# Chthi/Ofighters

Measured on AMD Instinct MI355X. Metric: arena-steps/sec (env.step+obs+policy fwd) at 4096 arenas, 1/2/4/8 MI355X, higher is better.
Workload: dtype f32; 1 GPU; 4096 arenas x 8 ships per GPU, random-bot actions + step + 2D obs rasterise (u8 maps) + bi-head policy forward for 8 ship(s)/arena, trunk shared per arena (BASELINE configs[3]); arenas_per_gpu=4096, ships=8, laser_cap=512, episode_ticks=200, parallelism=arena-sharded x1, RCCL all-reduce of episodic scores only, laser_overflow=0, last_episode_score_sum=70993, last_episode_arenas=4096

## Files before the change

ofighters_amd/csrc/ofx_head.hip:

```cpp
#include "ofx_head.h"
#include "ofx_lowp.h"
#include "ofx_diag.h"
#include <stdlib.h>


typedef float f32x4 __attribute__((ext_vector_type(4)));
typedef float f32x2 __attribute__((ext_vector_type(2)));
#define HD_PS 400
constexpr int HC4_ZERO = 800;
constexpr int HC4_COL = 816, HC4_CPITCH = 416;
constexpr int HC4_STRIDE = HC4_COL + 2 * HC4_CPITCH + 16;
__device__ __forceinline__ int hc4_at(int ln, int t) { return ln < 2 ? ln * 400 + t : HC4_COL + (ln - 2) * HC4_CPITCH + t; }
__device__ __forceinline__ int hc4_pad(int k) { return k < 16 ? HC4_ZERO + k : k < 32 ? HC4_COL + 400 + k - 16 : HC4_COL + HC4_CPITCH + 400 + k - 32; }

__device__ __forceinline__ void hc4_zero_block(const HeadParams2 &p, int tid, int threads) {
  if (blockIdx.x == 0)
    for (int e = tid; e < HC4_STRIDE; e += threads) p.c4[(size_t)p.S * HC4_STRIDE + e] = 0.f;
}

__device__ __forceinline__ float hd_max_raw(float x, float floor) {
  float pinf;
  asm("s_mov_b32 %0, 0x7f800000" : "=s"(pinf));
  return __builtin_amdgcn_fmed3f(x, floor, pinf);
}
// ... 182 lines not shown
    float acc = 0.f;
    if (!isc || (t > 0 && t < 399)) {
      const int d0 = side ? 2 : 0;
#pragma unroll
      for (int d1 = 0; d1 < 3; d1++)
#pragma unroll
        for (int ci = 0; ci < 8; ci++) {
          const int tap = isc ? d1 * 3 + d0 : d0 * 3 + d1;
          acc += p.w4raw[tap * 8 + ci] * hf_up(u3l + ln * 1600 + ci, 8, 200, t + d1 - 1, p.legacy);
        }
      if (!isc && (t == 0 || t == 399)) {
        const int cl = t ? 3 : 2, dx = t ? 2 : 0;
        for (int dy = 0; dy < 3; dy++) {
          if (dy == d0) continue;
          const int yy = (side ? 399 : 0) + dy - 1;
          if (yy < 0 || yy > 399) continue;
          for (int ci = 0; ci < 8; ci++) acc += p.w4raw[(dy * 3 + dx) * 8 + ci] * hf_up(u3l + cl * 1600 + ci, 8, 200, yy, p.legacy);
        }
      }
    }
    p.c4[(size_t)s * HC4_STRIDE + hc4_at(ln, t)] = acc;
  }
  if (tid < 64) p.c4[(size_t)s * HC4_STRIDE + hc4_pad(tid)] = 0.f;
}

constexpr int HG_THREADS = 256;
constexpr int HG_L1 = 0;
constexpr int HG_U3 = 0;
constexpr int HG_RB = 6400;
constexpr int HG_CB = HG_RB + 4 * 102 * 4;
constexpr int HG_TOTAL = HG_CB + 4 * 102 * 4;
static_assert(2 * 52 * 52 <= 6400, "l1p fits under u3l");

template <int CIN, int COUT, class G>
__device__ __forceinline__ float hg_corner(G get, int n, int yc, int xc, const float *w, float bias, int co, int legacy) {
  float acc = bias;
  for (int dy = 0; dy < 3; dy++) {
    const int uy = yc + dy - 1;
    if (uy < 0 || uy >= 2 * n) continue;
    int ya, yb; float wy;
    hf_taps(uy, n, ya, yb, wy, legacy);
    for (int dx = 0; dx < 3; dx++) {
      const int ux = xc + dx - 1;
      if (ux < 0 || ux >= 2 * n) continue;
      int xa, xb; float wx;
      hf_taps(ux, n, xa, xb, wx, legacy);
      for (int ci = 0; ci < CIN; ci++) {
        const float a = get(ya, xa, ci), b = get(ya, xb, ci), d = get(yb, xa, ci), g = get(yb, xb, ci);
        const float top = a + (b - a) * wx, bot = d + (g - d) * wx;
        acc += w[((dy * 3 + dx) * CIN + ci) * COUT + co] * (top + (bot - top) * wy);
      }
    }
  }
  return fmaxf(acc, 0.f);
}

__global__ __launch_bounds__(HG_THREADS) void k_head_frames(HeadParams2 p) {
  __shared__ __align__(16) float sm[HG_TOTAL];
  __shared__ float efr_s[192], w4s[72];
  const int s = hd_ship(p, (int)((blockIdx.x & ~7u) | ((blockIdx.x + (blockIdx.x >> 3)) & 7u)));
  const int tid = threadIdx.x, lane = tid & 63;
  hc4_zero_block(p, tid, HG_THREADS);
  if (s < 0) return;
  const int wv = __builtin_amdgcn_readfirstlane(tid >> 6);
  const int n16 = lane & 15, kq = lane >> 4;
  float *l1p = sm + HG_L1, *u2rb = sm + HG_RB, *u2cb = sm + HG_CB, *u3l = sm + HG_U3;

  {
    constexpr int NB = 6 * 52 + 46 * 6, NE = 2 * NB, PER = (NE + HG_THREADS - 1) / HG_THREADS;
    float v[PER];
    int at[PER];
#pragma unroll
    for (int u = 0; u < PER; u++) {
      const int e = min(u * HG_THREADS + tid, NE - 1);
      const int ci = e / NB, k = e - ci * NB;
      int r, c;
      if (k < 6 * 52) { const int rr = k / 52; r = rr < 3 ? rr : rr + 46; c = k - rr * 52; }
      else { const int k2 = k - 6 * 52, cc = k2 % 6; r = 3 + k2 / 6; c = cc < 3 ? cc : cc + 46; }
      at[u] = (ci * 52 + r) * 52 + c;
      v[u] = p.up1[(size_t)s * 5000 + (ci * 50 + min(max(r - 1, 0), 49)) * 50 + min(max(c - 1, 0), 49)];
    }
#pragma unroll
    for (int u = 0; u < PER; u++)
      if (u * HG_THREADS + tid < NE) l1p[at[u]] = v[u];
  }
  if (tid < 192) efr_s[tid] = p.efr[tid];
  if (tid < 72) w4s[tid] = p.w4raw[tid];
  __syncthreads();

  float bw2[5];
#pragma unroll
  for (int jj = 0; jj < 5; jj++) bw2[jj] = p.w2fr[(wv * 20 + 4 * jj + kq) * 16 + n16];
  float bw3[9];
#pragma unroll
  for (int jj = 0; jj < 9; jj++) bw3[jj] = p.w3fr[(wv * 36 + 4 * jj + kq) * 16 + n16];
#pragma unroll 1
  for (int m = 0; m < 4; m++) {
    const int v = wv;
    const int pp = min(16 * m + n16, 49);
    const int i = v == 0 ? 0 : v == 1 ? 49 : pp, j = v == 2 ? 0 : v == 3 ? 49 : pp;
    const float bias = p.b2[n16 & 3];
    f32x4 d = {bias, bias, bias, bias};
#pragma unroll
    for (int jj = 0; jj < 5; jj++) {
      const int tap = min(2 * jj + (kq >> 1), 8);
      const float a = l1p[((kq & 1) * 52 + i + tap / 3) * 52 + j + tap % 3];
      d = __builtin_amdgcn_mfma_f32_16x16x4f32(a, bw2[jj], d, 0, 0, 0);
    }
    const int co = n16 & 3, pa = n16 >> 3, pb = (n16 >> 2) & 1;
#pragma unroll
    for (int r = 0; r < 4; r++) {
      const int q = 16 * m + 4 * kq + r;
      if (q >= 50) continue;
      const float val = fmaxf(d[r], 0.f);
      if (v < 2) {
        u2rb[((2 * v + pa) * 102 + 2 * q + pb + 1) * 4 + co] = val;
      } else {
        u2cb[((2 * (v - 2) + pb) * 102 + 2 * q + pa + 1) * 4 + co] = val;
      }
    }
  }
  __syncthreads();
  if (tid < 64) {
    const int co = tid & 3, cx = (tid >> 2) & 1, cy = (tid >> 3) & 1, bx = (tid >> 4) & 1, by = tid >> 5;
    const int y = by ? 98 + cy : cy, x = bx ? 98 + cx : cx;
    const int rb = by ? 2 + cy : cy, cb = bx ? 2 + cx : cx;
    const bool fy = y == 0 || y == 99, fx = x == 0 || x == 99;
    float val;
    if (fy && fx) {
      auto get = [&](int yy, int xx, int ci) { return l1p[(ci * 52 + yy + 1) * 52 + xx + 1]; };
      val = hg_corner<2, 4>(get, 50, y, x, p.w2raw, p.b2[co], co, p.legacy);
    } else if (fx) {
      val = u2cb[(cb * 102 + y + 1) * 4 + co];
    } else {
      val = u2rb[(rb * 102 + x + 1) * 4 + co];
    }
    if (fy && fx) { u2rb[(rb * 102 + x + 1) * 4 + co] = val; u2cb[(cb * 102 + y + 1) * 4 + co] = val; }
    else if (fx) u2rb[(rb * 102 + x + 1) * 4 + co] = val;
    else u2cb[(cb * 102 + y + 1) * 4 + co] = val;
  }
  __syncthreads();
  if (tid < 128) {
    const int co = tid & 3, b = (tid >> 2) & 3, hi = (tid >> 4) & 1, isc = tid >> 5;
    if (isc < 2) {
      float *ln = (isc ? u2cb : u2rb) + b * 102 * 4;
      ln[(hi ? 101 : 0) * 4 + co] = ln[(hi ? 100 : 1) * 4 + co];
    }
  }
  for (int e = tid; e < 4 * 100 * 4; e += HG_THREADS) {
    const int ln = e / 400, r = e - ln * 400;
    const float *src = ln < 2 ? u2rb + (ln ? 3 : 0) * 408 : u2cb + (ln == 3 ? 3 : 0) * 408;
    p.u2fr[(size_t)s * 1600 + e] = src[4 + r];
  }
  __syncthreads();

#pragma unroll 1
  for (int m = 0; m < 7; m++) {
    const int v = wv;
    const int qq = min(16 * m + n16, 99);
    const float *band = (v < 2 ? u2rb : u2cb);
    const int b0 = (v & 1) ? 2 : 0;
    const float bias = p.b3[n16 & 7];
    f32x4 d = {bias, bias, bias, bias};
#pragma unroll
    for (int jj = 0; jj < 9; jj++) {
      const int ty = jj / 3, tx = jj % 3;
      const int tf = v < 2 ? ty : tx, ta = v < 2 ? tx : ty;
      const int bsel = (v & 1) ? b0 + min(tf, 1) : b0 + max(tf - 1, 0);
      const float a = band[(bsel * 102 + qq + ta) * 4 + kq];
      d = __builtin_amdgcn_mfma_f32_16x16x4f32(a, bw3[jj], d, 0, 0, 0);
    }
    const int co = n16 & 7, par = n16 >> 3;
#pragma unroll
    for (int r = 0; r < 4; r++) {
      const int q = 16 * m + 4 * kq + r;
      if (q < 100) u3l[(v * 200 + 2 * q + par) * 8 + co] = fmaxf(d[r], 0.f);
    }
  }
  __syncthreads();
  if (tid < 32) {
    const int co = tid & 7, c = tid >> 3;
    const int y = (c & 1) ? 199 : 0, x = (c & 2) ? 199 : 0;
    auto get = [&](int yy, int xx, int ci) {
      return u2rb[((yy < 50 ? yy : yy - 96) * 102 + xx + 1) * 4 + ci];
    };
    const float val = hg_corner<4, 8>(get, 100, y, x, p.w3raw, p.b3[co], co, p.legacy);
    u3l[(((c & 1) ? 1 : 0) * 200 + x) * 8 + co] = val;
    u3l[(((c & 2) ? 3 : 2) * 200 + y) * 8 + co] = val;
  }
  __syncthreads();
  if (tid < 252) {
    const int tp = tid % 9, c0 = tid / 9;
    float wt[8];
#pragma unroll
    for (int ci = 0; ci < 8; ci++) wt[ci] = w4s[tp * 8 + ci];
    float *dst = p.vfr + (size_t)s * 7200 + tid;
    for (int cell = c0; cell < 4 * 200; cell += 28) {
      const f32x4 ua = *reinterpret_cast<const f32x4 *>(u3l + cell * 8), ub = *reinterpret_cast<const f32x4 *>(u3l + cell * 8 + 4);
      float acc = 0.f;
#pragma unroll
      for (int ci = 0; ci < 4; ci++) acc = fmaf(wt[ci], ua[ci], acc);
#pragma unroll
      for (int ci = 0; ci < 4; ci++) acc = fmaf(wt[4 + ci], ub[ci], acc);
      dst[(cell - c0) * 9] = acc;
    }
  }

  for (int e = tid; e < 4 * 400; e += HG_THREADS) {
    const int ln = e / 400, t = e - ln * 400, isc = ln >> 1, side = ln & 1, jq = t >> 1, b = t & 1;
    float acc = 0.f;
    if (!isc || (t > 0 && t < 399)) {
      const float *E = efr_s + ((isc * 2 + side) * 2 + b) * 24;
      const float *L = u3l + ln * 1600;
#pragma unroll
      for (int o = 0; o < 3; o++) {
        const float *Lp = L + min(max(jq + o - 1, 0), 199) * 8;
#pragma unroll
        for (int ci = 0; ci < 8; ci++) acc += E[o * 8 + ci] * Lp[ci];
      }
      if (!isc && (t == 0 || t == 399)) {
        const int cs = t ? 1 : 0;
        const int yq = side ? 199 : 0, a = side ? 1 : 0;
        const float *E2 = efr_s + ((2 + cs) * 2 + a) * 24;
        const float *L2 = u3l + (2 + cs) * 1600;
        for (int o = 0; o < 3; o++) {
          const float *Lp = L2 + min(max(yq + o - 1, 0), 199) * 8;
          for (int ci = 0; ci < 8; ci++) acc += E2[o * 8 + ci] * Lp[ci];
        }
        const int tap = (side ? 2 : 0) * 3 + (cs ? 2 : 0);
        const float *Lc = L + (t ? 199 : 0) * 8;
        for (int ci = 0; ci < 8; ci++) acc -= p.w4raw[tap * 8 + ci] * Lc[ci];
      }
    }
    p.c4[(size_t)s * HC4_STRIDE + hc4_at(ln, t)] = acc;
  }
  if (tid < 64) p.c4[(size_t)s * HC4_STRIDE + hc4_pad(tid)] = 0.f;
}

constexpr int HS_GPR = 13;
constexpr int HS_NTILES = 325;
constexpr int HS_NS = 42;
constexpr int HS_NR3 = 16, HS_P3 = 106;
constexpr int HS_PL3 = HS_NR3 * HS_P3 + 4;
constexpr int HS_NV = 9;
constexpr int HS_NR2 = 16, HS_P2 = 56;
constexpr int HS_PL2 = (HS_NR2 + 2) * HS_P2;
static_assert(HS_PL2 % 32 == 16, "uprelu2 plane stride");
constexpr int HS_TABP = 16 * HS_GPR;
static_assert(HS_TABP == 4 * 52, "table period in tiles");
static_assert(4 * (HS_NV * HS_PL3 + 4 * HS_PL2 + HS_TABP + 400) <= 80 * 1024, "two workgroups per CU");
struct alignas(16) HsPick { signed char v[HS_NS][4]; };
constexpr int hs_pairs_done_c(int s) { return s + 2 + ((s + 2) >> 2) < 50 ? s + 2 + ((s + 2) >> 2) : 50; }
constexpr HsPick hs_make_pick() {
  HsPick t{};
  for (int st = 0; st < HS_NS; st++)
    for (int cw = 0; cw < 4; cw++) {
      const int lo = 2 * hs_pairs_done_c(st), hi = 2 * hs_pairs_done_c(st + 1);
      const int at = lo + ((cw - lo) & 3);
      t.v[st][cw] = (signed char)(at < hi ? at >> 1 : -1);
    }
  return t;
}
__constant__ HsPick kHsPick = hs_make_pick();

// ... 558 lines not shown
```

ofighters_amd/csrc/ofx_policy.hip:

```cpp
#include <string.h>

#include "ofx_internal.h"
#include "ofx_blob.h"
#include "ofx_trunk.h"
#include "ofx_head.h"

typedef float f32x16 __attribute__((ext_vector_type(16)));


extern "C" int ofx_policy_layout(const ofx_handle *h, ofx_policy_desc *desc) {
  (void)h;
  if (!desc) { ofx_set_error("ofx_policy_layout: null desc"); return OFX_ERR_INVALID; }
  memset(desc, 0, sizeof(*desc));
  desc->n_tensors = policy_layout(desc->offset, desc->count);
  desc->n_floats = desc->offset[desc->n_tensors];
  return OFX_OK;
}

struct PrepLayout {
  int tw[4], tb[4];
  int uw[3], ub[3];
  int w3mf;
  int w2mf;
  int w2fr;
  int w3fr;
  int w4eff_c;
  int w4raw;
  int efr;
  int b4;
  int zero16;
  int wbm[3];
  int lut1;
  int total;
};

static PrepLayout prep_layout() {
  PrepLayout L;
  int off = 0;
  for (int i = 0; i < 4; i++) { L.tw[i] = off; off += 9 * kTrunkCin[i] * 8; L.tb[i] = off; off += 8; }
  for (int i = 0; i < 3; i++) { L.uw[i] = off; off += 9 * kUpCin[i] * kUpCout[i]; L.ub[i] = off; off += kUpCout[i]; }
// ... 147 lines not shown
      p.prep[p.dst_wbm[l - 1] + e] = (tr >= 0 && tr < 3) ? p.prep[p.dst_w[l] + ((tr * 3 + dx) * 8 + ci) * 8 + co] : 0.f;
    }
  }
}

__global__ __launch_bounds__(256) void k_upconv1(ConvParams p) {
  __shared__ float u0s[625];
  __shared__ float up[52][53];
  const int tid = threadIdx.x;
  const int n_items = p.live ? p.live[0] : p.images;
#pragma unroll 1
  for (int it = blockIdx.x; it < n_items; it += gridDim.x) {
  const int img = p.live ? p.live[1 + it] : it;
  __syncthreads();
  for (int e = tid; e < 625; e += 256) u0s[e] = p.in[(size_t)img * 625 + e];
  __syncthreads();
  for (int e = tid; e < 52 * 52; e += 256) {
    const int c = e % 52, r = e / 52, gy = r - 1, gx = c - 1;
    float v = 0.f;
    if (gy >= 0 && gy < 50 && gx >= 0 && gx < 50) {
      const float sy = p.legacy ? (float)gy * 0.5f : ((float)gy + 0.5f) * 0.5f - 0.5f;
      const float sx = p.legacy ? (float)gx * 0.5f : ((float)gx + 0.5f) * 0.5f - 0.5f;
      const float fy = floorf(sy), fx = floorf(sx);
      const float ly = sy - fy, lx = sx - fx;
      int y0 = (int)fy, x0 = (int)fx, y1 = y0 + 1, x1 = x0 + 1;
      y0 = max(y0, 0); x0 = max(x0, 0); y1 = min(y1, 24); x1 = min(x1, 24);
      const float a = u0s[y0 * 25 + x0], b = u0s[y0 * 25 + x1], d = u0s[y1 * 25 + x0], g = u0s[y1 * 25 + x1];
      const float top = a + (b - a) * lx, bot = d + (g - d) * lx;
      v = top + (bot - top) * ly;
    }
    up[r][c] = v;
  }
  __syncthreads();
  if (tid < 250) {
  const int row = tid / 5, x0 = 10 * (tid - 5 * row);
  float acc[2][10];
#pragma unroll
  for (int co = 0; co < 2; co++)
#pragma unroll
    for (int i = 0; i < 10; i++) acc[co][i] = 0.f;
#pragma unroll
  for (int dy = 0; dy < 3; dy++) {
    float v[12];
#pragma unroll
    for (int i = 0; i < 12; i++) v[i] = up[row + dy][x0 + i];
#pragma unroll
    for (int dx = 0; dx < 3; dx++)
#pragma unroll
      for (int co = 0; co < 2; co++) {
        const float wv = p.w[(dy * 3 + dx) * 2 + co];
#pragma unroll
        for (int i = 0; i < 10; i++) acc[co][i] = __builtin_fmaf(v[i + dx], wv, acc[co][i]);
      }
  }
#pragma unroll
  for (int co = 0; co < 2; co++) {
    const float bias = p.b[co];
    float *o = p.out + (((size_t)img * 2 + co) * 50 + row) * 50 + x0;
#pragma unroll
    for (int i = 0; i < 10; i += 2)
      *reinterpret_cast<float2 *>(o + i) = make_float2(fmaxf(acc[co][i] + bias, 0.f), fmaxf(acc[co][i + 1] + bias, 0.f));
  }
  }
  }
}


__global__ __launch_bounds__(256) void k_gemm_f32(const float *A, int lda, const float *B, int ldb, const float *bias,
                                                  float *C, int ldc, int M, int N, int K, int relu, const int32_t *live) {
  const int lane = threadIdx.x & 63, wv = threadIdx.x >> 6;
  const int tiles_n = (N + 31) / 32;
  const int tile = blockIdx.x * 4 + wv;
  if (live) M = live[0];
  if (tile >= ((M + 31) / 32) * tiles_n) return;
  const int m0 = (tile / tiles_n) * 32, n0 = (tile % tiles_n) * 32;
  const int r0 = m0 + (lane & 31), c = n0 + (lane & 31), kh = lane >> 5;
  const bool rv = r0 < M, cv = c < N;
  const int r = live ? live[1 + (rv ? r0 : 0)] : r0;
  f32x16 acc;
#pragma unroll
  for (int i = 0; i < 16; i++) acc[i] = 0.f;
  const float *ap = A + (size_t)(rv ? r : 0) * lda + kh;
  const float *bp = B + (size_t)kh * ldb + (cv ? c : 0);
  for (int k0 = 0; k0 < K; k0 += 2) {
    const bool kv = k0 + kh < K;
    const float a = (rv && kv) ? ap[k0] : 0.f;
    const float b = (cv && kv) ? bp[(size_t)k0 * ldb] : 0.f;
    acc = __builtin_amdgcn_mfma_f32_32x32x2f32(a, b, acc, 0, 0, 0);
  }
  if (cv) {
    const float bv = bias ? bias[c] : 0.f;
#pragma unroll
    for (int i = 0; i < 16; i++) {
      const int row = m0 + (i & 3) + 8 * (i >> 2) + 4 * kh;
      if (row < M) {
        float v = acc[i] + bv;
        if (relu) v = fmaxf(v, 0.f);
        C[(size_t)(live ? live[1 + row] : row) * ldc + c] = v;
      }
    }
  }
}

__global__ __launch_bounds__(256) void k_gemm_f32_splitk(const float *A, int lda, const float *B, int ldb, float *P,
                                                         int M, int N, int Kc, int tiles, int jobs) {
  const int lane = threadIdx.x & 63, wv = threadIdx.x >> 6;
  const int tiles_n = (N + 31) / 32;
  const int job = blockIdx.x * 4 + wv;
  const int chunk = job / tiles, tile = job - chunk * tiles;
  if (job >= jobs) return;
  const int m0 = (tile / tiles_n) * 32, n0 = (tile % tiles_n) * 32;
  const int r = m0 + (lane & 31), c = n0 + (lane & 31), kh = lane >> 5;
  const bool rv = r < M, cv = c < N;
  f32x16 acc;
#pragma unroll
  for (int i = 0; i < 16; i++) acc[i] = 0.f;
  const float *ap = A + (size_t)(rv ? r : 0) * lda + (size_t)chunk * Kc + 4 * kh;
  const float *bp = B + ((size_t)chunk * Kc + 4 * kh) * ldb + (cv ? c : 0);
  for (int k0 = 0; k0 < Kc; k0 += 8) {
    const float4 a4 = *reinterpret_cast<const float4 *>(ap + k0);
    const float b0 = bp[(size_t)(k0 + 0) * ldb], b1 = bp[(size_t)(k0 + 1) * ldb], b2 = bp[(size_t)(k0 + 2) * ldb],
                b3 = bp[(size_t)(k0 + 3) * ldb];
    acc = __builtin_amdgcn_mfma_f32_32x32x2f32(rv ? a4.x : 0.f, cv ? b0 : 0.f, acc, 0, 0, 0);
    acc = __builtin_amdgcn_mfma_f32_32x32x2f32(rv ? a4.y : 0.f, cv ? b1 : 0.f, acc, 0, 0, 0);
    acc = __builtin_amdgcn_mfma_f32_32x32x2f32(rv ? a4.z : 0.f, cv ? b2 : 0.f, acc, 0, 0, 0);
    acc = __builtin_amdgcn_mfma_f32_32x32x2f32(rv ? a4.w : 0.f, cv ? b3 : 0.f, acc, 0, 0, 0);
  }
  if (cv) {
    float *out = P + (size_t)chunk * M * N;
#pragma unroll
    for (int i = 0; i < 16; i++) {
      const int row = m0 + (i & 3) + 8 * (i >> 2) + 4 * kh;
      if (row < M) out[(size_t)row * N + c] = acc[i];
    }
  }
}

struct HeadParams {
  int N, M;
  ofx_state st;
  const float *g1;
  int g1_chunks;
  const float *k1, *b1, *k2, *b2, *k3, *b3;
  const int32_t *live;
  const uint8_t *mask;
  const float *vec8;
  float *d1;
  float *act;
  int32_t *iaction;
};

__global__ __launch_bounds__(256) void k_head_dense(HeadParams p) {
  __shared__ float sd1[4][100];
  __shared__ float sd2[4][50];
  const int lane = threadIdx.x & 63, wv = threadIdx.x >> 6;
  const int item = blockIdx.x * 4 + wv, n_items = p.live ? p.live[0] : p.N * p.M;
  if ((int)blockIdx.x * 4 >= n_items) return;
  const bool on = item < n_items;
  const int s = on ? (p.live ? p.live[1 + item] : item) : 0;
  const int a = s / p.M;
  float vec[8];
  if (on) {
    if (p.vec8) {
#pragma unroll
      for (int k = 0; k < 8; k++) vec[k] = p.vec8[(size_t)s * 8 + k];
    } else {
      vec[0] = (float)p.st.reward[s]; vec[1] = 1.f;
      vec[2] = (float)p.st.ship_px[s]; vec[3] = (float)p.st.ship_py[s];
      vec[4] = (float)PS; vec[5] = (float)PS;
      vec[6] = (float)p.st.ship_x[s]; vec[7] = (float)p.st.ship_y[s];
    }
    for (int o = lane; o < 100; o += 64) {
      float acc = 0.f;
#pragma unroll
      for (int k = 0; k < 8; k++) acc += vec[k] * p.k1[k * 100 + o];
      float g = 0.f;
      for (int ch = 0; ch < p.g1_chunks; ch++) g += p.g1[((size_t)ch * p.N + a) * 100 + o];
      acc += g;
      acc += p.b1[o];
      acc = fmaxf(acc, 0.f);
      sd1[wv][o] = acc;
      p.d1[(size_t)s * 100 + o] = acc;
    }
  }
  __syncthreads();
  if (on && lane < 50) {
    float acc = 0.f;
    for (int k = 0; k < 100; k++) acc += sd1[wv][k] * p.k2[k * 50 + lane];
    sd2[wv][lane] = fmaxf(acc + p.b2[lane], 0.f);
  }
  __syncthreads();
  if (on && lane < 2) {
    float acc = 0.f;
    for (int k = 0; k < 50; k++) acc += sd2[wv][k] * p.k3[k * 2 + lane];
    acc += p.b3[lane];
    if (p.act) p.act[(size_t)s * 2 + lane] = acc;
    const float other = __shfl_xor(acc, 1);
    if (lane == 0 && p.iaction) p.iaction[s] = other > acc ? 1 : 0;
  }
}

__device__ inline float unordered_f32(unsigned o) {
  return __uint_as_float((o & 0x80000000u) ? (o & 0x7FFFFFFFu) : ~o);
}

__global__ void k_policy_finish(int S, const uint8_t *mask, const unsigned long long *best, int32_t *ipointer,
                                float *ptr_max) {
  const int s = blockIdx.x * blockDim.x + threadIdx.x;
  if (s >= S || (mask && !mask[s])) return;
  const bool none = best[s] == 0ull;
  const unsigned k = none ? 0u : ~(unsigned)(best[s] & 0xFFFFFFFFull);
  ipointer[2 * s] = (int)(k % PS);
  ipointer[2 * s + 1] = (int)(k / PS);
  if (ptr_max) ptr_max[s] = none ? __builtin_nanf("") : unordered_f32((unsigned)(best[s] >> 32));
}

__global__ void k_policy_actions(int S, const ofx_state st, const int32_t *iaction, const int32_t *ipointer,
                                 const uint8_t *mask, ofx_action *out) {
  const int s = blockIdx.x * blockDim.x + threadIdx.x;
  if (s >= S || (mask && !mask[s])) return;
  ofx_action a;
  a.valid = st.alive[s] ? 1 : 0;
  a.shoot = iaction[s] == 0;
  a.thrust = iaction[s] == 1;
  a.px = ipointer[2 * s];
  a.py = ipointer[2 * s + 1];
  a._pad = 0;
  out[s] = a;
}

struct PolicyWs {
// ... 120 lines not shown
  float *act_values, *heatmap, *ptr_max, *ptr_probe;
  int32_t *iaction, *ipointer;
  const int32_t *probe;
};

static int policy_forward_impl(ofx_handle *h, const ForwardArgs &a) {
  const int N = a.N, S = a.N * a.M;
  const float *weights = a.weights;
  PolicyWs ws;
  int rc = policy_workspace(h, &ws, N, S);
  if (rc) return rc;
  int32_t off[64], cnt[64];
  policy_layout(off, cnt);
  const PrepLayout L = prep_layout();

  const bool pinned = h->prep && h->prep_pinned == weights;
  if (!pinned && (rc = policy_prepare(h, weights, &h->prep_tmp))) return rc;
  const float *prep = pinned ? h->prep : h->prep_tmp;

  const int lowp = a.vec8 == nullptr ? h->opt_policy_lowp : 0;
  TrunkParams tp;
  memset(&tp, 0, sizeof(tp));
  tp.bits[0] = a.bits[0]; tp.bits[1] = a.bits[1]; tp.bits_stride = a.bits_stride; tp.images = N;
  for (int i = 0; i < 4; i++) { tp.tw[i] = prep + L.tw[i]; tp.tb[i] = prep + L.tb[i]; }
  for (int i = 0; i < 3; i++) tp.wbm[i] = prep + L.wbm[i];
  tp.lut1 = prep + L.lut1; tp.zero16 = prep + L.zero16;
  tp.p1 = ws.p1; tp.p2 = ws.p2; tp.p3 = ws.p3; tp.p4 = ws.p4;
  tp.lowp = lowp; tp.sparse = h->opt_trunk_sparse || a.vec8 != nullptr;
  tp.stat = h->opt_trunk_sparse ? h->trunk_stat : nullptr;
  if ((rc = ofx_launch_trunk(h, tp))) return rc;

  const float *k1 = weights + off[OFX_T_DENSE1];
  {
    const int tiles = ((N + 31) / 32) * 4, jobs = tiles * kDense1Chunks;
    hipLaunchKernelGGL(k_gemm_f32_splitk, dim3((jobs + 3) / 4), dim3(256), 0, h->stream, ws.p4, 5000, k1 + 8 * 100, 100,
                       ws.g1, N, 100, 5000 / kDense1Chunks, tiles, jobs);
    OFX_HIP(hipGetLastError());
  }
  HeadParams hp;
  hp.N = N; hp.M = a.M; hp.st = h->st; hp.vec8 = a.vec8; hp.g1 = ws.g1; hp.g1_chunks = kDense1Chunks;
  hp.k1 = k1; hp.b1 = weights + off[OFX_T_DENSE1 + 1];
  hp.k2 = weights + off[OFX_T_DENSE2]; hp.b2 = weights + off[OFX_T_DENSE2 + 1];
  hp.k3 = weights + off[OFX_T_OUT1]; hp.b3 = weights + off[OFX_T_OUT1 + 1];
  const int32_t *live = nullptr;
  if (a.ship_mask) {
    if ((rc = ofx_head_compact(h, S, a.ship_mask, ws.live))) return rc;
    live = ws.live;
  }
  hp.mask = a.ship_mask; hp.live = live; hp.d1 = ws.d1; hp.act = a.act_values; hp.iaction = a.iaction ? a.iaction : ws.iaction;
  hipLaunchKernelGGL(k_head_dense, dim3((S + 3) / 4), dim3(256), 0, h->stream, hp);
  OFX_HIP(hipGetLastError());

  if ((rc = ofx_launch_gemm(h, ws.d1, 100, weights + off[OFX_T_UPDENSE], 625, weights + off[OFX_T_UPDENSE + 1], ws.u0, 625, S, 625, 100, 1, live)))
    return rc;
  ConvParams up;
  memset(&up, 0, sizeof(up));
  up.live = live; up.images = S; up.legacy = h->opt_bilinear_legacy;
  up.in = ws.u0; up.w = prep + L.uw[0]; up.b = prep + L.ub[0]; up.out = ws.up1;
  hipLaunchKernelGGL(k_upconv1, dim3((unsigned)(live && S > 4096 ? 4096 : S)), dim3(256), 0, h->stream, up);
  OFX_HIP(hipGetLastError());
  OFX_HIP(hipMemsetAsync(ws.best, 0, sizeof(unsigned long long) * S, h->stream));
  HeadParams2 hp2;
  memset(&hp2, 0, sizeof(hp2));
  hp2.S = S; hp2.up1 = ws.up1;
  hp2.w2mf = prep + L.w2mf; hp2.b2 = prep + L.ub[1]; hp2.w2raw = prep + L.uw[1];
  hp2.w3mf = prep + L.w3mf; hp2.b3 = prep + L.ub[2]; hp2.w3raw = prep + L.uw[2];
  hp2.w4eff_c = prep + L.w4eff_c; hp2.b4 = prep + L.b4; hp2.w4raw = prep + L.w4raw;
  hp2.w2fr = prep + L.w2fr; hp2.w3fr = prep + L.w3fr; hp2.efr = prep + L.efr;
  hp2.u2fr = ws.u2fr; hp2.vfr = ws.vfr; hp2.c4 = ws.c4;
  hp2.frames_ref = h->opt_frames_ref; hp2.legacy = h->opt_bilinear_legacy;
  hp2.bf16 = lowp;
  hp2.mask = a.ship_mask; hp2.live = ws.live; hp2.live_ready = a.ship_mask != nullptr; hp2.best = ws.best; hp2.heat = a.heatmap;
  hp2.probe = a.probe; hp2.ptr_probe = a.probe ? a.ptr_probe : nullptr;
  const int pb = h->prof_base;
  hp2.event_base = pb;
  if ((rc = ofx_launch_head(h, hp2))) return rc;
  if (pb >= 0) h->prof_base = pb + 3 < OFX_RING_MAX ? pb + 2 : -1;
  hipLaunchKernelGGL(k_policy_finish, dim3((S + 255) / 256), dim3(256), 0, h->stream, S, a.ship_mask, ws.best,
                     a.ipointer ? a.ipointer : ws.ipointer, a.ptr_max);
  OFX_HIP(hipGetLastError());
  return OFX_OK;
}

extern "C" int ofx_policy_forward(ofx_handle *h, const float *weights, const uint8_t *ship_mask, float *act_values,
                                  int32_t *iaction, int32_t *ipointer, float *heatmap) {
  if (!h || !weights) { ofx_set_error("ofx_policy_forward: null argument"); return OFX_ERR_INVALID; }
  if (!h->spawned) { ofx_set_error("You must execute analyse_battleground first."); return OFX_ERR_STATE; }
  const ofx_config &c = h->cfg;
  if (c.width != PS || c.height != PS) {
    ofx_set_error("ofx_policy_forward: the pointer_model takes 400x400 maps (got %d x %d)", c.width, c.height);
    return OFX_ERR_INVALID;
  }
  OFX_HIP(hipSetDevice(c.device));
  int rc = ofx_launch_raster(h, OFX_MAP_BITS_LSB, nullptr, nullptr);
// ... 92 lines not shown
```

Measured before the change: 221,200 arena-steps/s.

## Restructure policy head GEMMs, dense head batching and head-frames MFMA loops

Rewrites the dense1 split-K GEMM to stage 64-row A tiles in LDS with register-prefetched B, and moves the chunk reduction into its own small kernel. Replaces the generic up-dense GEMM launch with a dedicated K=100 MFMA kernel that keeps A rows in LDS. Each k_head_dense wave now handles 8 ships, which reuses weight loads across them. Zeroing of `best` moves into that kernel, replacing a separate memset. Head-frames code interleaves two MFMA tiles per iteration, preloads corner weights into registers, reads w4 from LDS, and remaps upconv1 threads to cover all 256 lanes. The cost is more launches, higher register and LDS pressure, and `best` is now zeroed only for live ships.

```diff
diff --git a/ofighters_amd/csrc/ofx_head.hip b/ofighters_amd/csrc/ofx_head.hip
--- a/ofighters_amd/csrc/ofx_head.hip
+++ b/ofighters_amd/csrc/ofx_head.hip
@@ -238,23 +238,35 @@
 constexpr int HG_TOTAL = HG_CB + 4 * 102 * 4;
 static_assert(2 * 52 * 52 <= 6400, "l1p fits under u3l");
 
+template <int CIN, int COUT>
+__device__ __forceinline__ void hg_corner_w(float (&wt)[4 * CIN], int yc, int xc, const float *w, int co) {
+  const int dy0 = yc == 0 ? 1 : 0, dx0 = xc == 0 ? 1 : 0;
+#pragma unroll
+  for (int t = 0; t < 2; t++)
+#pragma unroll
+    for (int u = 0; u < 2; u++)
+#pragma unroll
+      for (int ci = 0; ci < CIN; ci++) wt[(t * 2 + u) * CIN + ci] = w[(((dy0 + t) * 3 + dx0 + u) * CIN + ci) * COUT + co];
+}
 template <int CIN, int COUT, class G>
-__device__ __forceinline__ float hg_corner(G get, int n, int yc, int xc, const float *w, float bias, int co, int legacy) {
+__device__ __forceinline__ float hg_corner(G get, int n, int yc, int xc, const float (&wt)[4 * CIN], float bias, int legacy) {
+  const int dy0 = yc == 0 ? 1 : 0, dx0 = xc == 0 ? 1 : 0;
   float acc = bias;
-  for (int dy = 0; dy < 3; dy++) {
-    const int uy = yc + dy - 1;
-    if (uy < 0 || uy >= 2 * n) continue;
+#pragma unroll
+  for (int t = 0; t < 2; t++) {
+    const int uy = yc + dy0 + t - 1;
     int ya, yb; float wy;
     hf_taps(uy, n, ya, yb, wy, legacy);
-    for (int dx = 0; dx < 3; dx++) {
-      const int ux = xc + dx - 1;
-      if (ux < 0 || ux >= 2 * n) continue;
+#pragma unroll
+    for (int u = 0; u < 2; u++) {
+      const int ux = xc + dx0 + u - 1;
       int xa, xb; float wx;
       hf_taps(ux, n, xa, xb, wx, legacy);
+#pragma unroll
       for (int ci = 0; ci < CIN; ci++) {
         const float a = get(ya, xa, ci), b = get(ya, xb, ci), d = get(yb, xa, ci), g = get(yb, xb, ci);
         const float top = a + (b - a) * wx, bot = d + (g - d) * wx;
-        acc += w[((dy * 3 + dx) * CIN + ci) * COUT + co] * (top + (bot - top) * wy);
+        acc += wt[(t * 2 + u) * CIN + ci] * (top + (bot - top) * wy);
       }
     }
   }
@@ -292,39 +304,63 @@
   }
   if (tid < 192) efr_s[tid] = p.efr[tid];
   if (tid < 72) w4s[tid] = p.w4raw[tid];
-  __syncthreads();
-
   float bw2[5];
 #pragma unroll
   for (int jj = 0; jj < 5; jj++) bw2[jj] = p.w2fr[(wv * 20 + 4 * jj + kq) * 16 + n16];
   float bw3[9];
 #pragma unroll
   for (int jj = 0; jj < 9; jj++) bw3[jj] = p.w3fr[(wv * 36 + 4 * jj + kq) * 16 + n16];
+  const float bias2 = p.b2[n16 & 3], bias3 = p.b3[n16 & 7];
+  float wc2[8], wc3[16], bc2 = 0.f, bc3 = 0.f;
+#pragma unroll
+  for (int e = 0; e < 8; e++) wc2[e] = 0.f;
+#pragma unroll
+  for (int e = 0; e < 16; e++) wc3[e] = 0.f;
+  if (tid < 64 && ((tid >> 3) & 1) == (tid >> 5) && ((tid >> 2) & 1) == ((tid >> 4) & 1)) {
+    hg_corner_w<2, 4>(wc2, (tid >> 5) ? 99 : 0, ((tid >> 4) & 1) ? 99 : 0, p.w2raw, tid & 3);
+    bc2 = p.b2[tid & 3];
+  }
+  if (tid < 32) {
+    hg_corner_w<4, 8>(wc3, ((tid >> 3) & 1) ? 199 : 0, ((tid >> 3) & 2) ? 199 : 0, p.w3raw, tid & 7);
+    bc3 = p.b3[tid & 7];
+  }
+  __syncthreads();
+
 #pragma unroll 1
-  for (int m = 0; m < 4; m++) {
+  for (int m0 = 0; m0 < 4; m0 += 2) {
     const int v = wv;
-    const int pp = min(16 * m + n16, 49);
-    const int i = v == 0 ? 0 : v == 1 ? 49 : pp, j = v == 2 ? 0 : v == 3 ? 49 : pp;
-    const float bias = p.b2[n16 & 3];
-    f32x4 d = {bias, bias, bias, bias};
+    f32x4 d[2];
+    int ai[2];
+#pragma unroll
+    for (int c = 0; c < 2; c++) {
+      const int pp = min(16 * (m0 + c) + n16, 49);
+      const int i = v == 0 ? 0 : v == 1 ? 49 : pp, j = v == 2 ? 0 : v == 3 ? 49 : pp;
+      ai[c] = ((kq & 1) * 52 + i) * 52 + j;
+      d[c] = f32x4{bias2, bias2, bias2, bias2};
+    }
 #pragma unroll
     for (int jj = 0; jj < 5; jj++) {
       const int tap = min(2 * jj + (kq >> 1), 8);
-      const float a = l1p[((kq & 1) * 52 + i + tap / 3) * 52 + j + tap % 3];
-      d = __builtin_amdgcn_mfma_f32_16x16x4f32(a, bw2[jj], d, 0, 0, 0);
+#pragma unroll
+      for (int c = 0; c < 2; c++) {
+        const float a = l1p[ai[c] + (tap / 3) * 52 + tap % 3];
+        d[c] = __builtin_amdgcn_mfma_f32_16x16x4f32(a, bw2[jj], d[c], 0, 0, 0);
+      }
     }
     const int co = n16 & 3, pa = n16 >> 3, pb = (n16 >> 2) & 1;
 #pragma unroll
-    for (int r = 0; r < 4; r++) {
-      const int q = 16 * m + 4 * kq + r;
-      if (q >= 50) continue;
-      const float val = fmaxf(d[r], 0.f);
-      if (v < 2) {
-        u2rb[((2 * v + pa) * 102 + 2 * q + pb + 1) * 4 + co] = val;
-      } else {
-        u2cb[((2 * (v - 2) + pb) * 102 + 2 * q + pa + 1) * 4 + co] = val;
-      }
-    }
+    for (int c = 0; c < 2; c++)
+#pragma unroll
+      for (int r = 0; r < 4; r++) {
+        const int q = 16 * (m0 + c) + 4 * kq + r;
+        if (q >= 50) continue;
+        const float val = fmaxf(d[c][r], 0.f);
+        if (v < 2) {
+          u2rb[((2 * v + pa) * 102 + 2 * q + pb + 1) * 4 + co] = val;
+        } else {
+          u2cb[((2 * (v - 2) + pb) * 102 + 2 * q + pa + 1) * 4 + co] = val;
+        }
+      }
   }
   __syncthreads();
   if (tid < 64) {
@@ -335,7 +371,7 @@
     float val;
     if (fy && fx) {
       auto get = [&](int yy, int xx, int ci) { return l1p[(ci * 52 + yy + 1) * 52 + xx + 1]; };
-      val = hg_corner<2, 4>(get, 50, y, x, p.w2raw, p.b2[co], co, p.legacy);
+      val = hg_corner<2, 4>(get, 50, y, x, wc2, bc2, p.legacy);
     } else if (fx) {
       val = u2cb[(cb * 102 + y + 1) * 4 + co];
     } else {
@@ -361,27 +397,31 @@
   __syncthreads();
 
 #pragma unroll 1
-  for (int m = 0; m < 7; m++) {
+  for (int m0 = 0; m0 < 8; m0 += 2) {
     const int v = wv;
-    const int qq = min(16 * m + n16, 99);
     const float *band = (v < 2 ? u2rb : u2cb);
     const int b0 = (v & 1) ? 2 : 0;
-    const float bias = p.b3[n16 & 7];
-    f32x4 d = {bias, bias, bias, bias};
+    f32x4 d[2] = {f32x4{bias3, bias3, bias3, bias3}, f32x4{bias3, bias3, bias3, bias3}};
 #pragma unroll
     for (int jj = 0; jj < 9; jj++) {
       const int ty = jj / 3, tx = jj % 3;
       const int tf = v < 2 ? ty : tx, ta = v < 2 ? tx : ty;
       const int bsel = (v & 1) ? b0 + min(tf, 1) : b0 + max(tf - 1, 0);
-      const float a = band[(bsel * 102 + qq + ta) * 4 + kq];
-      d = __builtin_amdgcn_mfma_f32_16x16x4f32(a, bw3[jj], d, 0, 0, 0);
+#pragma unroll
+      for (int c = 0; c < 2; c++) {
+        const int qq = min(16 * (m0 + c) + n16, 99);
+        const float a = band[(bsel * 102 + qq + ta) * 4 + kq];
+        d[c] = __builtin_amdgcn_mfma_f32_16x16x4f32(a, bw3[jj], d[c], 0, 0, 0);
+      }
     }
     const int co = n16 & 7, par = n16 >> 3;
 #pragma unroll
-    for (int r = 0; r < 4; r++) {
-      const int q = 16 * m + 4 * kq + r;
-      if (q < 100) u3l[(v * 200 + 2 * q + par) * 8 + co] = fmaxf(d[r], 0.f);
-    }
+    for (int c = 0; c < 2; c++)
+#pragma unroll
+      for (int r = 0; r < 4; r++) {
+        const int q = 16 * (m0 + c) + 4 * kq + r;
+        if (q < 100) u3l[(v * 200 + 2 * q + par) * 8 + co] = fmaxf(d[c][r], 0.f);
+      }
   }
   __syncthreads();
   if (tid < 32) {
@@ -390,7 +430,7 @@
     auto get = [&](int yy, int xx, int ci) {
       return u2rb[((yy < 50 ? yy : yy - 96) * 102 + xx + 1) * 4 + ci];
     };
-    const float val = hg_corner<4, 8>(get, 100, y, x, p.w3raw, p.b3[co], co, p.legacy);
+    const float val = hg_corner<4, 8>(get, 100, y, x, wc3, bc3, p.legacy);
     u3l[(((c & 1) ? 1 : 0) * 200 + x) * 8 + co] = val;
     u3l[(((c & 2) ? 3 : 2) * 200 + y) * 8 + co] = val;
   }
@@ -435,7 +475,7 @@
         }
         const int tap = (side ? 2 : 0) * 3 + (cs ? 2 : 0);
         const float *Lc = L + (t ? 199 : 0) * 8;
-        for (int ci = 0; ci < 8; ci++) acc -= p.w4raw[tap * 8 + ci] * Lc[ci];
+        for (int ci = 0; ci < 8; ci++) acc -= w4s[tap * 8 + ci] * Lc[ci];
       }
     }
     p.c4[(size_t)s * HC4_STRIDE + hc4_at(ln, t)] = acc;
diff --git a/ofighters_amd/csrc/ofx_policy.hip b/ofighters_amd/csrc/ofx_policy.hip
--- a/ofighters_amd/csrc/ofx_policy.hip
+++ b/ofighters_amd/csrc/ofx_policy.hip
@@ -6,6 +6,8 @@
 #include "ofx_head.h"
 
 typedef float f32x16 __attribute__((ext_vector_type(16)));
+typedef float f32x4 __attribute__((ext_vector_type(4)));
+typedef float f32x2 __attribute__((ext_vector_type(2)));
 
 
 extern "C" int ofx_policy_layout(const ofx_handle *h, ofx_policy_desc *desc) {
@@ -219,35 +221,30 @@
     up[r][c] = v;
   }
   __syncthreads();
-  if (tid < 250) {
-  const int row = tid / 5, x0 = 10 * (tid - 5 * row);
-  float acc[2][10];
-#pragma unroll
-  for (int co = 0; co < 2; co++)
-#pragma unroll
-    for (int i = 0; i < 10; i++) acc[co][i] = 0.f;
-#pragma unroll
-  for (int dy = 0; dy < 3; dy++) {
-    float v[12];
-#pragma unroll
-    for (int i = 0; i < 12; i++) v[i] = up[row + dy][x0 + i];
-#pragma unroll
-    for (int dx = 0; dx < 3; dx++)
-#pragma unroll
-      for (int co = 0; co < 2; co++) {
-        const float wv = p.w[(dy * 3 + dx) * 2 + co];
-#pragma unroll
-        for (int i = 0; i < 10; i++) acc[co][i] = __builtin_fmaf(v[i + dx], wv, acc[co][i]);
-      }
-  }
-#pragma unroll
-  for (int co = 0; co < 2; co++) {
-    const float bias = p.b[co];
-    float *o = p.out + (((size_t)img * 2 + co) * 50 + row) * 50 + x0;
-#pragma unroll
-    for (int i = 0; i < 10; i += 2)
-      *reinterpret_cast<float2 *>(o + i) = make_float2(fmaxf(acc[co][i] + bias, 0.f), fmaxf(acc[co][i + 1] + bias, 0.f));
-  }
+#pragma unroll 1
+  for (int e = tid; e < 1250; e += 256) {
+    const int row = e / 25, x0 = 2 * (e - 25 * row);
+    float acc[2][2] = {{0.f, 0.f}, {0.f, 0.f}};
+#pragma unroll
+    for (int dy = 0; dy < 3; dy++) {
+      float v[4];
+#pragma unroll
+      for (int i = 0; i < 4; i++) v[i] = up[row + dy][x0 + i];
+#pragma unroll
+      for (int dx = 0; dx < 3; dx++)
+#pragma unroll
+        for (int co = 0; co < 2; co++) {
+          const float wv = p.w[(dy * 3 + dx) * 2 + co];
+#pragma unroll
+          for (int i = 0; i < 2; i++) acc[co][i] = __builtin_fmaf(v[i + dx], wv, acc[co][i]);
+        }
+    }
+#pragma unroll
+    for (int co = 0; co < 2; co++) {
+      const float bias = p.b[co];
+      *reinterpret_cast<float2 *>(p.out + ((size_t)img * 2 + co) * 2500 + 2 * e) =
+          make_float2(fmaxf(acc[co][0] + bias, 0.f), fmaxf(acc[co][1] + bias, 0.f));
+    }
   }
   }
 }
@@ -289,45 +286,172 @@
   }
 }
 
+constexpr int AR_P = 52;
+template <int K, int NT>
+__device__ __forceinline__ void gemm_arows_tiles(const float *ar, const float *B, int ldb, const float *bias, float *C,
+                                                 int ldc, int M, int N, int relu, const int32_t *live, int m0, int lane, int t0) {
+  const int kh = lane >> 5;
+  f32x16 acc[NT];
+  const float *bp[NT];
+  bool cv[NT];
+#pragma unroll
+  for (int q = 0; q < NT; q++) {
+    const int c = (t0 + 4 * q) * 32 + (lane & 31);
+    cv[q] = c < N;
+    bp[q] = B + (size_t)kh * ldb + (cv[q] ? c : 0);
+#pragma unroll
+    for (int i = 0; i < 16; i++) acc[q][i] = 0.f;
+  }
+#pragma unroll 2
+  for (int i4 = 0; i4 < K / 8; i4++) {
+    const f32x4 x = *reinterpret_cast<const f32x4 *>(ar + 4 * i4);
+#pragma unroll
+    for (int u = 0; u < 4; u++)
+#pragma unroll
+      for (int q = 0; q < NT; q++) {
+        const float b = cv[q] ? bp[q][(size_t)(2 * u) * ldb] : 0.f;
+        acc[q] = __builtin_amdgcn_mfma_f32_32x32x2f32(x[u], b, acc[q], 0, 0, 0);
+      }
+#pragma unroll
+    for (int q = 0; q < NT; q++) bp[q] += (size_t)8 * ldb;
+  }
+  {
+    const f32x2 x = *reinterpret_cast<const f32x2 *>(ar + 4 * (K / 8));
+#pragma unroll
+    for (int u = 0; u < 2; u++)
+#pragma unroll
+      for (int q = 0; q < NT; q++) {
+        const float b = cv[q] ? bp[q][(size_t)(2 * u) * ldb] : 0.f;
+        acc[q] = __builtin_amdgcn_mfma_f32_32x32x2f32(x[u], b, acc[q], 0, 0, 0);
+      }
+  }
+#pragma unroll
+  for (int q = 0; q < NT; q++) {
+    if (!cv[q]) continue;
+    const int c = (t0 + 4 * q) * 32 + (lane & 31);
+    const float bv = bias ? bias[c] : 0.f;
+#pragma unroll
+    for (int i = 0; i < 16; i++) {
+      const int row = m0 + (i & 3) + 8 * (i >> 2) + 4 * kh;
+      if (row < M) {
+        float v = acc[q][i] + bv;
+        if (relu) v = fmaxf(v, 0.f);
+        C[(size_t)(live ? live[1 + row] : row) * ldc + c] = v;
+      }
+    }
+  }
+}
+
+template <int K>
+__global__ __launch_bounds__(256) __attribute__((amdgpu_waves_per_eu(4, 4)))
+void k_gemm_f32_arows(const float *A, int lda, const float *B, int ldb, const float *bias, float *C, int ldc, int M, int N,
+                      int relu, const int32_t *live) {
+  static_assert(K % 8 == 4 && K / 2 + 2 <= AR_P, "k_gemm_f32_arows: K");
+  __shared__ __align__(16) float sA[2 * 32 * AR_P];
+  const int tid = threadIdx.x, lane = tid & 63, wv = __builtin_amdgcn_readfirstlane(tid >> 6);
+  if (live) M = live[0];
+  const int m0 = blockIdx.x * 32;
+  if (m0 >= M) return;
+  {
+    constexpr int Q = K / 4, NE = 32 * Q, PER = (NE + 255) / 256;
+    float4 v[PER];
+#pragma unroll
+    for (int u = 0; u < PER; u++) {
+      const int e = min(u * 256 + tid, NE - 1), rr = e / Q, row = m0 + rr;
+      v[u] = make_float4(0.f, 0.f, 0.f, 0.f);
+      if (row < M) v[u] = *reinterpret_cast<const float4 *>(A + (size_t)(live ? live[1 + row] : row) * lda + 4 * (e - rr * Q));
+    }
+#pragma unroll
+    for (int u = 0; u < PER; u++) {
+      const int e = u * 256 + tid, rr = e / Q, i = 2 * (e - rr * Q);
+      if (e < NE) {
+        *reinterpret_cast<f32x2 *>(sA + rr * AR_P + i) = f32x2{v[u].x, v[u].z};
+        *reinterpret_cast<f32x2 *>(sA + (32 + rr) * AR_P + i) = f32x2{v[u].y, v[u].w};
+      }
+    }
+  }
+  __syncthreads();
+  const float *ar = sA + ((lane >> 5) * 32 + (lane & 31)) * AR_P;
+  const int tiles_n = (N + 31) / 32;
+  for (int t0 = wv; t0 < tiles_n; t0 += 8) {
+    if (t0 + 4 < tiles_n) gemm_arows_tiles<K, 2>(ar, B, ldb, bias, C, ldc, M, N, relu, live, m0, lane, t0);
+    else gemm_arows_tiles<K, 1>(ar, B, ldb, bias, C, ldc, M, N, relu, live, m0, lane, t0);
+  }
+}
+
+constexpr int SK_KC = 200, SK_P = SK_KC + 4;
 __global__ __launch_bounds__(256) void k_gemm_f32_splitk(const float *A, int lda, const float *B, int ldb, float *P,
-                                                         int M, int N, int Kc, int tiles, int jobs) {
-  const int lane = threadIdx.x & 63, wv = threadIdx.x >> 6;
-  const int tiles_n = (N + 31) / 32;
-  const int job = blockIdx.x * 4 + wv;
-  const int chunk = job / tiles, tile = job - chunk * tiles;
-  if (job >= jobs) return;
-  const int m0 = (tile / tiles_n) * 32, n0 = (tile % tiles_n) * 32;
-  const int r = m0 + (lane & 31), c = n0 + (lane & 31), kh = lane >> 5;
-  const bool rv = r < M, cv = c < N;
-  f32x16 acc;
-#pragma unroll
-  for (int i = 0; i < 16; i++) acc[i] = 0.f;
-  const float *ap = A + (size_t)(rv ? r : 0) * lda + (size_t)chunk * Kc + 4 * kh;
+                                                         int M, int N, int Kc, int tiles_m64) {
+  __shared__ __align__(16) float sA[64 * SK_P];
+  const int tid = threadIdx.x, lane = tid & 63, wv = __builtin_amdgcn_readfirstlane(tid >> 6);
+  const int chunk = blockIdx.x / tiles_m64, m0 = (blockIdx.x - chunk * tiles_m64) * 64;
+  {
+    const int Q = Kc / 4, NE = 64 * Q;
+    constexpr int PER = (64 * (SK_KC / 4) + 255) / 256;
+    float4 v[PER];
+#pragma unroll
+    for (int u = 0; u < PER; u++) {
+      const int e = min(u * 256 + tid, NE - 1), rr = e / Q, row = m0 + rr;
+      v[u] = make_float4(0.f, 0.f, 0.f, 0.f);
+      if (row < M) v[u] = *reinterpret_cast<const float4 *>(A + (size_t)row * lda + (size_t)chunk * Kc + 4 * (e - rr * Q));
+    }
+#pragma unroll
+    for (int u = 0; u < PER; u++) {
+      const int e = u * 256 + tid, rr = e / Q;
+      if (e < NE) *reinterpret_cast<float4 *>(sA + rr * SK_P + 4 * (e - rr * Q)) = v[u];
+    }
+  }
+  __syncthreads();
+  const int c = wv * 32 + (lane & 31), kh = lane >> 5;
+  if (wv * 32 >= N) return;
+  const bool cv = c < N;
+  f32x16 acc0, acc1;
+#pragma unroll
+  for (int i = 0; i < 16; i++) { acc0[i] = 0.f; acc1[i] = 0.f; }
+  const float *a0 = sA + (lane & 31) * SK_P + 4 * kh, *a1 = a0 + 32 * SK_P;
   const float *bp = B + ((size_t)chunk * Kc + 4 * kh) * ldb + (cv ? c : 0);
+  float b[4], bn[4];
+#pragma unroll
+  for (int j = 0; j < 4; j++) b[j] = cv ? bp[(size_t)j * ldb] : 0.f;
   for (int k0 = 0; k0 < Kc; k0 += 8) {
-    const float4 a4 = *reinterpret_cast<const float4 *>(ap + k0);
-    const float b0 = bp[(size_t)(k0 + 0) * ldb], b1 = bp[(size_t)(k0 + 1) * ldb], b2 = bp[(size_t)(k0 + 2) * ldb],
-                b3 = bp[(size_t)(k0 + 3) * ldb];
-    acc = __builtin_amdgcn_mfma_f32_32x32x2f32(rv ? a4.x : 0.f, cv ? b0 : 0.f, acc, 0, 0, 0);
-    acc = __builtin_amdgcn_mfma_f32_32x32x2f32(rv ? a4.y : 0.f, cv ? b1 : 0.f, acc, 0, 0, 0);
-    acc = __builtin_amdgcn_mfma_f32_32x32x2f32(rv ? a4.z : 0.f, cv ? b2 : 0.f, acc, 0, 0, 0);
-    acc = __builtin_amdgcn_mfma_f32_32x32x2f32(rv ? a4.w : 0.f, cv ? b3 : 0.f, acc, 0, 0, 0);
+    const int kn = min(k0 + 8, Kc - 8);
+#pragma unroll
+    for (int j = 0; j < 4; j++) bn[j] = cv ? bp[(size_t)(kn + j) * ldb] : 0.f;
+    const float4 x = *reinterpret_cast<const float4 *>(a0 + k0), y = *reinterpret_cast<const float4 *>(a1 + k0);
+    acc0 = __builtin_amdgcn_mfma_f32_32x32x2f32(x.x, b[0], acc0, 0, 0, 0);
+    acc1 = __builtin_amdgcn_mfma_f32_32x32x2f32(y.x, b[0], acc1, 0, 0, 0);
+    acc0 = __builtin_amdgcn_mfma_f32_32x32x2f32(x.y, b[1], acc0, 0, 0, 0);
+    acc1 = __builtin_amdgcn_mfma_f32_32x32x2f32(y.y, b[1], acc1, 0, 0, 0);
+    acc0 = __builtin_amdgcn_mfma_f32_32x32x2f32(x.z, b[2], acc0, 0, 0, 0);
+    acc1 = __builtin_amdgcn_mfma_f32_32x32x2f32(y.z, b[2], acc1, 0, 0, 0);
+    acc0 = __builtin_amdgcn_mfma_f32_32x32x2f32(x.w, b[3], acc0, 0, 0, 0);
+    acc1 = __builtin_amdgcn_mfma_f32_32x32x2f32(y.w, b[3], acc1, 0, 0, 0);
+#pragma unroll
+    for (int j = 0; j < 4; j++) b[j] = bn[j];
   }
   if (cv) {
     float *out = P + (size_t)chunk * M * N;
 #pragma unroll
     for (int i = 0; i < 16; i++) {
       const int row = m0 + (i & 3) + 8 * (i >> 2) + 4 * kh;
-      if (row < M) out[(size_t)row * N + c] = acc[i];
-    }
-  }
+      if (row < M) out[(size_t)row * N + c] = acc0[i];
+      if (row + 32 < M) out[(size_t)(row + 32) * N + c] = acc1[i];
+    }
+  }
+}
+
+__global__ __launch_bounds__(256) void k_dense1_reduce(float *g1, int n, int chunks) {
+  const int e = blockIdx.x * 256 + threadIdx.x;
+  if (e >= n) return;
+  float g = 0.f;
+  for (int ch = 0; ch < chunks; ch++) g += g1[(size_t)ch * n + e];
+  g1[e] = g;
 }
 
 struct HeadParams {
   int N, M;
   ofx_state st;
   const float *g1;
-  int g1_chunks;
   const float *k1, *b1, *k2, *b2, *k3, *b3;
   const int32_t *live;
   const uint8_t *mask;
@@ -335,55 +459,82 @@
   float *d1;
   float *act;
   int32_t *iaction;
+  unsigned long long *best;
 };
 
+constexpr int HD_SH = 8;
 __global__ __launch_bounds__(256) void k_head_dense(HeadParams p) {
-  __shared__ float sd1[4][100];
-  __shared__ float sd2[4][50];
-  const int lane = threadIdx.x & 63, wv = threadIdx.x >> 6;
-  const int item = blockIdx.x * 4 + wv, n_items = p.live ? p.live[0] : p.N * p.M;
-  if ((int)blockIdx.x * 4 >= n_items) return;
-  const bool on = item < n_items;
-  const int s = on ? (p.live ? p.live[1 + item] : item) : 0;
-  const int a = s / p.M;
-  float vec[8];
-  if (on) {
-    if (p.vec8) {
-#pragma unroll
-      for (int k = 0; k < 8; k++) vec[k] = p.vec8[(size_t)s * 8 + k];
-    } else {
-      vec[0] = (float)p.st.reward[s]; vec[1] = 1.f;
-      vec[2] = (float)p.st.ship_px[s]; vec[3] = (float)p.st.ship_py[s];
-      vec[4] = (float)PS; vec[5] = (float)PS;
-      vec[6] = (float)p.st.ship_x[s]; vec[7] = (float)p.st.ship_y[s];
-    }
-    for (int o = lane; o < 100; o += 64) {
-      float acc = 0.f;
-#pragma unroll
-      for (int k = 0; k < 8; k++) acc += vec[k] * p.k1[k * 100 + o];
-      float g = 0.f;
-      for (int ch = 0; ch < p.g1_chunks; ch++) g += p.g1[((size_t)ch * p.N + a) * 100 + o];
-      acc += g;
-      acc += p.b1[o];
-      acc = fmaxf(acc, 0.f);
-      sd1[wv][o] = acc;
-      p.d1[(size_t)s * 100 + o] = acc;
-    }
-  }
+  __shared__ __align__(16) float svec[4][8][HD_SH];
+  __shared__ __align__(16) float sd1[4][100][HD_SH];
+  __shared__ __align__(16) float sd2[4][50][HD_SH];
+  const int lane = threadIdx.x & 63, wv = __builtin_amdgcn_readfirstlane(threadIdx.x >> 6);
+  const int item0 = (blockIdx.x * 4 + wv) * HD_SH, n_items = p.live ? p.live[0] : p.N * p.M;
+  if ((int)blockIdx.x * 4 * HD_SH >= n_items) return;
+  {
+    const int j = lane >> 3, k = lane & 7;
+    float v = 0.f;
+    if (item0 + j < n_items) {
+      const int s = p.live ? p.live[1 + item0 + j] : item0 + j;
+      if (p.vec8) v = p.vec8[(size_t)s * 8 + k];
+      else v = k == 0 ? (float)p.st.reward[s] : k == 1 ? 1.f : k == 2 ? (float)p.st.ship_px[s] : k == 3 ? (float)p.st.ship_py[s]
+             : k < 6 ? (float)PS : k == 6 ? (float)p.st.ship_x[s] : (float)p.st.ship_y[s];
+      if (k == 0 && p.best) p.best[s] = 0ull;
+    }
+    svec[wv][k][j] = v;
+  }
+  int sh[HD_SH];
+#pragma unroll
+  for (int j = 0; j < HD_SH; j++) sh[j] = item0 + j < n_items ? (p.live ? p.live[1 + item0 + j] : item0 + j) : -1;
   __syncthreads();
-  if (on && lane < 50) {
+  for (int o = lane; o < 100; o += 64) {
+    float acc[HD_SH];
+#pragma unroll
+    for (int j = 0; j < HD_SH; j++) acc[j] = 0.f;
+#pragma unroll
+    for (int k = 0; k < 8; k++) {
+      const float w = p.k1[k * 100 + o];
+#pragma unroll
+      for (int j = 0; j < HD_SH; j++) acc[j] += svec[wv][k][j] * w;
+    }
+    const float b1 = p.b1[o];
+#pragma unroll
+    for (int j = 0; j < HD_SH; j++) {
+      float v = 0.f;
+      if (sh[j] >= 0) {
+        v = acc[j];
+        v += p.g1[(size_t)(sh[j] / p.M) * 100 + o];
+        v += b1;
+        v = fmaxf(v, 0.f);
+        p.d1[(size_t)sh[j] * 100 + o] = v;
+      }
+      sd1[wv][o][j] = v;
+    }
+  }
+  __syncthreads();
+  if (lane < 50) {
+    float acc[HD_SH];
+#pragma unroll
+    for (int j = 0; j < HD_SH; j++) acc[j] = 0.f;
+#pragma unroll 4
+    for (int k = 0; k < 100; k++) {
+      const float w = p.k2[k * 50 + lane];
+#pragma unroll
+      for (int j = 0; j < HD_SH; j++) acc[j] += sd1[wv][k][j] * w;
+    }
+    const float b2 = p.b2[lane];
+#pragma unroll
+    for (int j = 0; j < HD_SH; j++) sd2[wv][lane][j] = fmaxf(acc[j] + b2, 0.f);
+  }
+  __syncthreads();
+  if (lane < 2 * HD_SH) {
+    const int j = lane >> 1, o = lane & 1;
+    const int s = item0 + j < n_items ? (p.live ? p.live[1 + item0 + j] : item0 + j) : -1;
     float acc = 0.f;
-    for (int k = 0; k < 100; k++) acc += sd1[wv][k] * p.k2[k * 50 + lane];
-    sd2[wv][lane] = fmaxf(acc + p.b2[lane], 0.f);
-  }
-  __syncthreads();
-  if (on && lane < 2) {
-    float acc = 0.f;
-    for (int k = 0; k < 50; k++) acc += sd2[wv][k] * p.k3[k * 2 + lane];
-    acc += p.b3[lane];
-    if (p.act) p.act[(size_t)s * 2 + lane] = acc;
+    for (int k = 0; k < 50; k++) acc += sd2[wv][k][j] * p.k3[k * 2 + o];
+    acc += p.b3[o];
+    if (s >= 0 && p.act) p.act[(size_t)s * 2 + o] = acc;
     const float other = __shfl_xor(acc, 1);
-    if (lane == 0 && p.iaction) p.iaction[s] = other > acc ? 1 : 0;
+    if (s >= 0 && o == 0 && p.iaction) p.iaction[s] = other > acc ? 1 : 0;
   }
 }
 
@@ -570,13 +721,15 @@
 
   const float *k1 = weights + off[OFX_T_DENSE1];
   {
-    const int tiles = ((N + 31) / 32) * 4, jobs = tiles * kDense1Chunks;
-    hipLaunchKernelGGL(k_gemm_f32_splitk, dim3((jobs + 3) / 4), dim3(256), 0, h->stream, ws.p4, 5000, k1 + 8 * 100, 100,
-                       ws.g1, N, 100, 5000 / kDense1Chunks, tiles, jobs);
+    static_assert(5000 / kDense1Chunks == SK_KC && 5000 % kDense1Chunks == 0, "dense1 chunk");
+    const int tiles_m64 = (N + 63) / 64;
+    hipLaunchKernelGGL(k_gemm_f32_splitk, dim3(tiles_m64 * kDense1Chunks), dim3(256), 0, h->stream, ws.p4, 5000, k1 + 8 * 100, 100,
+                       ws.g1, N, 100, SK_KC, tiles_m64);
+    hipLaunchKernelGGL(k_dense1_reduce, dim3((N * 100 + 255) / 256), dim3(256), 0, h->stream, ws.g1, N * 100, kDense1Chunks);
     OFX_HIP(hipGetLastError());
   }
   HeadParams hp;
-  hp.N = N; hp.M = a.M; hp.st = h->st; hp.vec8 = a.vec8; hp.g1 = ws.g1; hp.g1_chunks = kDense1Chunks;
+  hp.N = N; hp.M = a.M; hp.st = h->st; hp.vec8 = a.vec8; hp.g1 = ws.g1;
   hp.k1 = k1; hp.b1 = weights + off[OFX_T_DENSE1 + 1];
   hp.k2 = weights + off[OFX_T_DENSE2]; hp.b2 = weights + off[OFX_T_DENSE2 + 1];
   hp.k3 = weights + off[OFX_T_OUT1]; hp.b3 = weights + off[OFX_T_OUT1 + 1];
@@ -586,18 +739,19 @@
     live = ws.live;
   }
   hp.mask = a.ship_mask; hp.live = live; hp.d1 = ws.d1; hp.act = a.act_values; hp.iaction = a.iaction ? a.iaction : ws.iaction;
-  hipLaunchKernelGGL(k_head_dense, dim3((S + 3) / 4), dim3(256), 0, h->stream, hp);
+  hp.best = ws.best;
+  hipLaunchKernelGGL(k_head_dense, dim3((S + 4 * HD_SH - 1) / (4 * HD_SH)), dim3(256), 0, h->stream, hp);
   OFX_HIP(hipGetLastError());
 
-  if ((rc = ofx_launch_gemm(h, ws.d1, 100, weights + off[OFX_T_UPDENSE], 625, weights + off[OFX_T_UPDENSE + 1], ws.u0, 625, S, 625, 100, 1, live)))
-    return rc;
+  hipLaunchKernelGGL(k_gemm_f32_arows<100>, dim3((S + 31) / 32), dim3(256), 0, h->stream, ws.d1, 100, weights + off[OFX_T_UPDENSE], 625,
+                     weights + off[OFX_T_UPDENSE + 1], ws.u0, 625, S, 625, 1, live);
+  OFX_HIP(hipGetLastError());
   ConvParams up;
   memset(&up, 0, sizeof(up));
   up.live = live; up.images = S; up.legacy = h->opt_bilinear_legacy;
   up.in = ws.u0; up.w = prep + L.uw[0]; up.b = prep + L.ub[0]; up.out = ws.up1;
   hipLaunchKernelGGL(k_upconv1, dim3((unsigned)(live && S > 4096 ? 4096 : S)), dim3(256), 0, h->stream, up);
   OFX_HIP(hipGetLastError());
-  OFX_HIP(hipMemsetAsync(ws.best, 0, sizeof(unsigned long long) * S, h->stream));
   HeadParams2 hp2;
   memset(&hp2, 0, sizeof(hp2));
   hp2.S = S; hp2.up1 = ws.up1;
```

Result: no change. 222,300 arena-steps/s, median of 6 (+0.5%).
